# mishapadidar/GP-Derivatives-Variational-Inference

Hardware: AMD Instinct MI355X
Metric: ELBO steps/sec, DSVGP d=20 N=1M M=500 p=5 (higher is better)
Workload: dtype f32 (f64 Cholesky/solves); 1 GPU; DSVGP d=20 N=1M M=500 p=5 B=4096; global_batch=4096, per_gpu_batch=4096, M_prime=3000, parallelism=dp1 rows, trsm_nb=4096, graph_replay=False, one_call_step=True, dense_product=hand-written (gemm32.hip, v_mfma_f32_32x32x2_f32)

## Files before the change

gp-derivatives-variational-inference_amd/csrc/gemm32.hip:

```cpp
#include <cstdlib>
#include <type_traits>

#include "common.h"

namespace {

using acc16 = float __attribute__((ext_vector_type(16)));
using acc4f = float __attribute__((ext_vector_type(4)));
constexpr int TM = 128, TN = 128;

#ifndef G32_BK
#define G32_BK 32
#endif
#ifndef G32_MINW
#define G32_MINW 3
#endif
#ifndef G32_BAND
#define G32_BAND 8
#endif
#ifndef G32_DMA_BK
#define G32_DMA_BK 32
#endif
#ifndef G32_MF
#define G32_MF 32
#endif
#ifndef G32_SK_BELOW
#define G32_SK_BELOW 4096
#endif
#ifndef G32_SK_MINK
#define G32_SK_MINK 512
#endif
#ifndef G32_WIDE_ROUNDS
#define G32_WIDE_ROUNDS 3
#endif
#ifndef G32_WIDE_FILL
#define G32_WIDE_FILL 90
#endif
#ifndef G32_SK_SLOTS
#define G32_SK_SLOTS 256
#endif

struct G32 {
    const float* A; const float* B; float* C;
    int64_t lda, ldb, ldc;
    int M, N, K, tiles_m, tiles_n, flags, splitk, kslice, ntiles;
    float alpha;
    float* slab;
};

template <int BK, bool KC>
struct Stage {
    static constexpr int NV = BK / 8;
    float4 v[NV];
};

template <int BK>
struct FetchKC {
    static constexpr int CPR = BK / 4, RPP = 256 / CPR, NV = BK / 8;
    const float* P;
    int rowoff[NV];
    int kc, klim;
    __device__ __forceinline__ void init(const float* P_, int64_t ld, int mn0, int MN, int K, int tid) {
        P = P_;
        kc = (tid % CPR) * 4;
        klim = ((K + 3) / 4) * 4 - 4;
#pragma unroll
        for (int i = 0; i < NV; ++i) rowoff[i] = (int)(min(mn0 + tid / CPR + i * RPP, MN - 1) * ld);
    }
    __device__ __forceinline__ void load(int k0, int kend, Stage<BK, true>& s) const {
        const int k = k0 + kc;
        const float* p = P + min(k, klim);
#pragma unroll
        for (int i = 0; i < NV; ++i) s.v[i] = *reinterpret_cast<const float4*>(p + rowoff[i]);
        if (k0 + BK > kend) {
#pragma unroll
            for (int i = 0; i < NV; ++i) {
                s.v[i].x = (k < kend) ? s.v[i].x : 0.f;
                s.v[i].y = (k + 1 < kend) ? s.v[i].y : 0.f;
                s.v[i].z = (k + 2 < kend) ? s.v[i].z : 0.f;
                s.v[i].w = (k + 3 < kend) ? s.v[i].w : 0.f;
            }
        }
    }
};
template <int BK>
struct FetchMC {
    static constexpr int NV = BK / 8;
    const float* P;
    int64_t ld;
    int kr, K;
    __device__ __forceinline__ void init(const float* P_, int64_t ld_, int mn0, int MN, int K_, int tid) {
        ld = ld_; K = K_;
        kr = tid >> 5;
        P = P_ + min(mn0 + (tid & 31) * 4, ((MN + 3) / 4) * 4 - 4);
    }
    __device__ __forceinline__ void load(int k0, int kend, Stage<BK, false>& s) const {
#pragma unroll
        for (int i = 0; i < NV; ++i) {
            const int k = k0 + kr + 8 * i;
            s.v[i] = *reinterpret_cast<const float4*>(P + (int64_t)min(k, K - 1) * ld);
            if (k0 + BK > kend && k >= kend) s.v[i] = float4{0.f, 0.f, 0.f, 0.f};
        }
    }
};

template <int TM_ = TM, int TN_ = TN>
__device__ __forceinline__ bool pick_unit(const G32& g, int& m0, int& n0, int& kbeg, int& kend) {
    const int u = (blockIdx.x >> 3) + (blockIdx.x & 7) * ((gridDim.x + 7) >> 3);
    if (u >= g.ntiles * g.splitk) return false;
    const int slice = u / g.ntiles;
    const int t = u - slice * g.ntiles;
    int tm, tn;
    if (g.flags & DSVGP_GEMM_OUT_LOWER) {
        const int tri = min(g.tiles_m, g.tiles_n), t0 = tri * (tri + 1) / 2;
        if (t < t0) {
            tm = (int)((sqrtf(8.f * (float)t + 1.f) - 1.f) * 0.5f);
            while ((tm + 1) * (tm + 2) / 2 <= t) ++tm;
            while (tm * (tm + 1) / 2 > t) --tm;
            tn = t - tm * (tm + 1) / 2;
        } else {
            tm = tri + (t - t0) / g.tiles_n;
            tn = (t - t0) % g.tiles_n;
        }
    } else {
        const int band = t / (G32_BAND * g.tiles_m), q = t - band * G32_BAND * g.tiles_m;
        const int wcols = min(G32_BAND, g.tiles_n - band * G32_BAND);
        tm = q / wcols;
        tn = band * G32_BAND + q - tm * wcols;
    }
    m0 = tm * TM_; n0 = tn * TN_;
    kbeg = slice * g.kslice; kend = min(g.K, kbeg + g.kslice);
    return true;
}

template <int NI, int NJ>
__device__ __forceinline__ void store_tile(const G32& g, const acc16 (&acc)[NI][NJ], int m0, int n0, int wr, int wc, int h, int r,
                                           float* Cb, int64_t ldcb, bool atomic_) {
    const bool atomic = atomic_, out_lower = g.flags & DSVGP_GEMM_OUT_LOWER;
#pragma unroll
    for (int i = 0; i < NI; ++i)
#pragma unroll
        for (int j = 0; j < NJ; ++j)
#pragma unroll
            for (int c = 0; c < 16; ++c) {
                const int m = m0 + wr * (32 * NI) + i * 32 + (c & 3) + 8 * (c >> 2) + 4 * h;
                const int n = n0 + wc * (32 * NJ) + j * 32 + r;
                if (m >= g.M || n >= g.N) continue;
                if (out_lower && n > m) continue;
                const float v = g.alpha * acc[i][j][c];
                float* dst = Cb + (int64_t)m * ldcb + n;
                if (atomic) atomicAdd(dst, v);
                else *dst = v;
            }
}
#define G32_DEST()                                                                                     \
    const int slice_ = g.kslice > 0 ? kbeg / g.kslice : 0;                                             \
    float* const Cb = g.slab ? g.slab + (int64_t)slice_ * g.M * g.N : g.C;                            \
    const int64_t ldcb = g.slab ? (int64_t)g.N : g.ldc;                                                \
    const bool atomic_ = g.splitk > 1 && !g.slab

template <int BK, bool A_KC, bool B_KC>
__global__ __launch_bounds__(256, G32_MINW) void gemm32_kernel(const G32 g) {
    constexpr int SKC = BK + 2, SMC = TM + 4;
    constexpr int A_WORDS = A_KC ? TM * SKC : BK * SMC, B_WORDS = B_KC ? TN * SKC : BK * SMC;
    __shared__ __attribute__((aligned(16))) float lds[A_WORDS + B_WORDS];
    float* As = lds;
    float* Bs = lds + A_WORDS;
    const int tid = threadIdx.x, lane = tid & 63, wave = tid >> 6, wr = wave >> 1, wc = wave & 1;
    const int h = lane >> 5, r = lane & 31;
    int m0, n0, kbeg, kend;
    if (!pick_unit(g, m0, n0, kbeg, kend)) return;

    Stage<BK, A_KC> ra;
    Stage<BK, B_KC> rb;
    typename std::conditional<A_KC, FetchKC<BK>, FetchMC<BK>>::type fa;
    typename std::conditional<B_KC, FetchKC<BK>, FetchMC<BK>>::type fb;
    fa.init(g.A, g.lda, m0, g.M, g.K, tid);
    fb.init(g.B, g.ldb, n0, g.N, g.K, tid);
    auto fetch = [&](int k0) {
        fa.load(k0, kend, ra);
        fb.load(k0, kend, rb);
    };
    auto commit = [&]() {
        if constexpr (A_KC) {
            constexpr int CPR = BK / 4, RPP = 256 / CPR;
            float* p = As + (tid / CPR) * SKC + (tid % CPR) * 4;
#pragma unroll
            for (int i = 0; i < BK / 8; ++i) {
                *reinterpret_cast<float2*>(p + i * RPP * SKC) = float2{ra.v[i].x, ra.v[i].y};
                *reinterpret_cast<float2*>(p + i * RPP * SKC + 2) = float2{ra.v[i].z, ra.v[i].w};
            }
        } else {
            float* p = As + (tid >> 5) * SMC + (tid & 31) * 4;
#pragma unroll
            for (int i = 0; i < BK / 8; ++i) *reinterpret_cast<float4*>(p + 8 * i * SMC) = ra.v[i];
        }
        if constexpr (B_KC) {
            constexpr int CPR = BK / 4, RPP = 256 / CPR;
            float* p = Bs + (tid / CPR) * SKC + (tid % CPR) * 4;
#pragma unroll
            for (int i = 0; i < BK / 8; ++i) {
                *reinterpret_cast<float2*>(p + i * RPP * SKC) = float2{rb.v[i].x, rb.v[i].y};
                *reinterpret_cast<float2*>(p + i * RPP * SKC + 2) = float2{rb.v[i].z, rb.v[i].w};
            }
        } else {
            float* p = Bs + (tid >> 5) * SMC + (tid & 31) * 4;
#pragma unroll
            for (int i = 0; i < BK / 8; ++i) *reinterpret_cast<float4*>(p + 8 * i * SMC) = rb.v[i];
        }
    };

    acc16 acc[2][2];
#pragma unroll
    for (int i = 0; i < 2; ++i)
#pragma unroll
        for (int j = 0; j < 2; ++j)
#pragma unroll
            for (int c = 0; c < 16; ++c) acc[i][j][c] = 0.f;

    const float* af = A_KC ? As + (wr * 64 + r) * SKC + 2 * h : As + (2 * h) * SMC + wr * 64 + r;
    const float* bf = B_KC ? Bs + (wc * 64 + r) * SKC + 2 * h : Bs + (2 * h) * SMC + wc * 64 + r;

    if (kbeg < kend) {
        fetch(kbeg);
        for (int k0 = kbeg; k0 < kend; k0 += BK) {
            commit();
            __syncthreads();
            if (k0 + BK < kend) fetch(k0 + BK);
#pragma unroll
            for (int kk = 0; kk < BK / 4; ++kk) {
                float2 a[2], b[2];
#pragma unroll
                for (int i = 0; i < 2; ++i) {
                    if constexpr (A_KC) a[i] = *reinterpret_cast<const float2*>(af + i * 32 * SKC + 4 * kk);
                    else a[i] = float2{af[(4 * kk) * SMC + i * 32], af[(4 * kk + 1) * SMC + i * 32]};
                }
#pragma unroll
                for (int j = 0; j < 2; ++j) {
                    if constexpr (B_KC) b[j] = *reinterpret_cast<const float2*>(bf + j * 32 * SKC + 4 * kk);
                    else b[j] = float2{bf[(4 * kk) * SMC + j * 32], bf[(4 * kk + 1) * SMC + j * 32]};
                }
#pragma unroll
                for (int i = 0; i < 2; ++i)
#pragma unroll
                    for (int j = 0; j < 2; ++j) {
                        acc[i][j] = __builtin_amdgcn_mfma_f32_32x32x2f32(a[i].x, b[j].x, acc[i][j], 0, 0, 0);
                        acc[i][j] = __builtin_amdgcn_mfma_f32_32x32x2f32(a[i].y, b[j].y, acc[i][j], 0, 0, 0);
                    }
            }
            __syncthreads();
        }
    }

    G32_DEST();
    store_tile(g, acc, m0, n0, wr, wc, h, r, Cb, ldcb, atomic_);
}

#ifdef G32_STAMP
__device__ unsigned long long g32_stamps[8];
#define G32_T(var) unsigned long long var; do { __builtin_amdgcn_sched_barrier(0); \
    asm volatile("s_memtime %0\n\ts_waitcnt lgkmcnt(0)" : "=s"(var) :: "memory"); __builtin_amdgcn_sched_barrier(0); } while (0)
#else
#define G32_T(var) do { } while (0)
#endif
typedef __attribute__((address_space(3))) void* lds_ptr_t;
typedef const __attribute__((address_space(1))) void* glb_ptr_t;
__device__ __attribute__((aligned(16))) float g32_zero_chunk[4] = {0.f, 0.f, 0.f, 0.f};

__device__ __forceinline__ void lds_dma16(const float* gsrc, unsigned lds_byte_addr) {
    unsigned keep;
    asm volatile("s_mov_b32 %0, m0\n\ts_mov_b32 m0, %2\n\ts_nop 0\n\tglobal_load_lds_dwordx4 %1, off\n\ts_mov_b32 m0, %0"
                 : "=&s"(keep) : "v"(gsrc), "s"(lds_byte_addr) : "memory");
}

template <int MF, bool A_KC, bool B_KC, int BK>
__global__ __launch_bounds__(256, BK == 16 ? 3 : 2) void gemm32_dma_kernel(const G32 g) {
    static_assert(BK == 32 || (BK == 16 && MF == 32), "the 64-byte-row swizzle is derived for the 32 x 32 x 2 shape");
    constexpr int OPW = 128 * BK;
    constexpr int NP = BK / 8;
    constexpr int CH = BK / 4, RPP = 256 / BK;
    constexpr int TS = MF, NT = 64 / TS, NH = 64 / TS, NJ = BK / (4 * NH);
    __shared__ __attribute__((aligned(16))) float lds[2][2 * OPW];
    const int tid = threadIdx.x, lane = tid & 63, wave = tid >> 6, wr = wave >> 1, wc = wave & 1;
    const int h = lane / TS, r = lane % TS;
    int m0, n0, kbeg, kend;
    if (!pick_unit(g, m0, n0, kbeg, kend)) return;

    const float* asrc[NP];
    const float* bsrc[NP];
    int akk[NP], bkk[NP];
    const int K4 = (g.K + 3) / 4 * 4;
    auto swz = [](int R) { return BK == 32 ? ((R >> 1) & 7) : ((R >> 2) & 3); };
#pragma unroll
    for (int i = 0; i < NP; ++i) {
        const int blk = wave * NP + i;
        if constexpr (A_KC) {
            const int R = blk * RPP + lane / CH, c = (lane % CH) ^ swz(R);
            asrc[i] = g.A + (int64_t)min(m0 + R, g.M - 1) * g.lda + kbeg + 4 * c;
            akk[i] = 4 * c;
        } else {
            const int k = blk * 2 + (lane >> 5);
            asrc[i] = g.A + (int64_t)(kbeg + k) * g.lda + min(m0 + 4 * (lane & 31), (g.M + 3) / 4 * 4 - 4);
            akk[i] = k;
        }
        if constexpr (B_KC) {
            const int R = blk * RPP + lane / CH, c = (lane % CH) ^ swz(R);
            bsrc[i] = g.B + (int64_t)min(n0 + R, g.N - 1) * g.ldb + kbeg + 4 * c;
            bkk[i] = 4 * c;
        } else {
            const int k = blk * 2 + (lane >> 5);
            bsrc[i] = g.B + (int64_t)(kbeg + k) * g.ldb + min(n0 + 4 * (lane & 31), (g.N + 3) / 4 * 4 - 4);
            bkk[i] = k;
        }
    }
    const int64_t astep = A_KC ? BK : (int64_t)BK * g.lda, bstep = B_KC ? BK : (int64_t)BK * g.ldb;
    const unsigned lds_base = (unsigned)(uintptr_t)(lds_ptr_t)&lds[0][0];
    const unsigned wave_u = __builtin_amdgcn_readfirstlane(wave);
    auto dma = [&](int buf, int k0) {
        const unsigned dst = lds_base + (unsigned)buf * (2 * OPW * 4) + wave_u * (NP * 1024);
        const bool tail = k0 + BK > kend;
#pragma unroll
        for (int i = 0; i < NP; ++i) {
            const float* sa = asrc[i];
            const float* sb = bsrc[i];
            if (tail) {
                if (k0 + akk[i] >= (A_KC ? K4 : g.K)) sa = g32_zero_chunk;
                if (k0 + bkk[i] >= (B_KC ? K4 : g.K)) sb = g32_zero_chunk;
            }
            lds_dma16(sa, dst + i * 1024);
            lds_dma16(sb, dst + OPW * 4 + i * 1024);
            asrc[i] += astep;
            bsrc[i] += bstep;
        }
    };

    using accT = typename std::conditional<MF == 32, acc16, acc4f>::type;
    accT acc[NT][NT];
#pragma unroll
    for (int i = 0; i < NT; ++i)
#pragma unroll
        for (int j = 0; j < NT; ++j)
#pragma unroll
            for (int c = 0; c < (MF == 32 ? 16 : 4); ++c) acc[i][j][c] = 0.f;

    const int q7 = h ^ swz(r);
    int aoff[NJ], boff[NJ];
#pragma unroll
    for (int j = 0; j < NJ; ++j) {
        aoff[j] = A_KC ? (wr * 64 + r) * BK + 4 * ((NH * j) ^ q7) : (4 * NH * j + 4 * h) * 128 + wr * 64 + r;
        boff[j] = B_KC ? (wc * 64 + r) * BK + 4 * ((NH * j) ^ q7) : (4 * NH * j + 4 * h) * 128 + wc * 64 + r;
    }

    struct Frag { float a[NT][4], b[NT][4]; };
    auto load_frag = [&](const float* As, const float* Bs, int j, Frag& f) {
#pragma unroll
        for (int i = 0; i < NT; ++i) {
            if constexpr (A_KC) {
                const float4 v = *reinterpret_cast<const float4*>(As + aoff[j] + i * TS * BK);
                f.a[i][0] = v.x; f.a[i][1] = v.y; f.a[i][2] = v.z; f.a[i][3] = v.w;
            } else {
#pragma unroll
                for (int e = 0; e < 4; ++e) f.a[i][e] = As[aoff[j] + e * 128 + i * TS];
            }
            if constexpr (B_KC) {
                const float4 v = *reinterpret_cast<const float4*>(Bs + boff[j] + i * TS * BK);
                f.b[i][0] = v.x; f.b[i][1] = v.y; f.b[i][2] = v.z; f.b[i][3] = v.w;
            } else {
#pragma unroll
                for (int e = 0; e < 4; ++e) f.b[i][e] = Bs[boff[j] + e * 128 + i * TS];
            }
        }
    };

    if (kbeg < kend) {
        dma(0, kbeg);
        asm volatile("s_waitcnt vmcnt(0)" ::: "memory");
        __syncthreads();
        int buf = 0;
#ifdef G32_STAMP
        unsigned long long d_dma = 0, d_mfma = 0, d_vm = 0, d_bar = 0, n_st = 0;
#endif
        for (int k0 = kbeg; k0 < kend; k0 += BK, buf ^= 1) {
            G32_T(t0);
            if (k0 + BK < kend) dma(buf ^ 1, k0 + BK);
            G32_T(t1);
            const float* As = &lds[buf][0];
            const float* Bs = As + OPW;
            Frag f[2];
            load_frag(As, Bs, 0, f[0]);
#pragma unroll
            for (int j = 0; j < NJ; ++j) {
                if (j + 1 < NJ) load_frag(As, Bs, j + 1, f[(j + 1) & 1]);
                __builtin_amdgcn_sched_barrier(0);
                const Frag& c = f[j & 1];
#pragma unroll
                for (int e = 0; e < 4; ++e)
#pragma unroll
                    for (int i = 0; i < NT; ++i)
#pragma unroll
                        for (int jn = 0; jn < NT; ++jn) {
                            if constexpr (MF == 32)
                                acc[i][jn] = __builtin_amdgcn_mfma_f32_32x32x2f32(c.a[i][e], c.b[jn][e], acc[i][jn], 0, 0, 0);
                            else
                                acc[i][jn] = __builtin_amdgcn_mfma_f32_16x16x4f32(c.a[i][e], c.b[jn][e], acc[i][jn], 0, 0, 0);
                        }
                __builtin_amdgcn_sched_barrier(0);
            }
            G32_T(t2);
            asm volatile("s_waitcnt vmcnt(0)" ::: "memory");
            G32_T(t3);
            __syncthreads();
#ifdef G32_STAMP
            G32_T(t4);
            d_dma += t1 - t0; d_mfma += t2 - t1; d_vm += t3 - t2; d_bar += t4 - t3; ++n_st;
#endif
        }
#ifdef G32_STAMP
        if (tid == 0 && blockIdx.x == gridDim.x / 2 + 8) {
            g32_stamps[0] = d_dma; g32_stamps[1] = d_mfma; g32_stamps[2] = d_vm; g32_stamps[3] = d_bar; g32_stamps[4] = n_st;
        }
#endif
    }
    G32_DEST();
    if constexpr (MF == 32) {
        store_tile(g, acc, m0, n0, wr, wc, h, r, Cb, ldcb, atomic_);
    } else {
        const bool atomic = atomic_, out_lower = g.flags & DSVGP_GEMM_OUT_LOWER;
#pragma unroll
        for (int i = 0; i < NT; ++i)
#pragma unroll
            for (int j = 0; j < NT; ++j)
#pragma unroll
                for (int c = 0; c < 4; ++c) {
                    const int m = m0 + wr * 64 + i * 16 + 4 * h + c;
                    const int n = n0 + wc * 64 + j * 16 + r;
                    if (m >= g.M || n >= g.N) continue;
                    if (out_lower && n > m) continue;
                    const float v = g.alpha * acc[i][j][c];
                    float* dst = Cb + (int64_t)m * ldcb + n;
                    if (atomic) atomicAdd(dst, v);
                    else *dst = v;
                }
    }
}

constexpr int WTM = 256, WTN = 192, WBK = 32;
constexpr int W_AWORDS = WTM * WBK, W_BWORDS = WBK * WTN, W_STAGE = W_AWORDS + W_BWORDS;
constexpr int W_NA = W_AWORDS / 1024, W_NB = W_BWORDS / 1024;
constexpr int W_LDS_BYTES = 2 * W_STAGE * 4;

__global__ __launch_bounds__(256, 1) void gemm32_wide_kernel(const G32 g) {
    extern __shared__ __attribute__((aligned(16))) float wlds[];
    const int tid = threadIdx.x, lane = tid & 63, wave = tid >> 6, wr = wave >> 1, wc = wave & 1;
    const int h = lane >> 5, r = lane & 31;
    int m0, n0, kbeg, kend;
    if (!pick_unit<WTM, WTN>(g, m0, n0, kbeg, kend)) return;

    const float* asrc[W_NA];
    const float* bsrc[W_NB];
    int akk[W_NA], bkk[W_NB];
    const int K4 = (g.K + 3) / 4 * 4;
#pragma unroll
    for (int i = 0; i < W_NA; ++i) {
        const int R = (wave * W_NA + i) * 8 + (lane >> 3), c = (lane & 7) ^ ((R >> 1) & 7);
        asrc[i] = g.A + (int64_t)min(m0 + R, g.M - 1) * g.lda + kbeg + 4 * c;
        akk[i] = 4 * c;
    }
#pragma unroll
    for (int i = 0; i < W_NB; ++i) {
        const int ch = (wave * W_NB + i) * 64 + lane, k = ch / (WTN / 4), n4 = ch % (WTN / 4);
        bsrc[i] = g.B + (int64_t)(kbeg + k) * g.ldb + min(n0 + 4 * n4, (g.N + 3) / 4 * 4 - 4);
        bkk[i] = k;
    }
    const int64_t bstep = (int64_t)WBK * g.ldb;
    const unsigned lds_base = (unsigned)(uintptr_t)(lds_ptr_t)&wlds[0];
    const unsigned wave_u = __builtin_amdgcn_readfirstlane(wave);

    acc16 acc[4][3];
#pragma unroll
    for (int i = 0; i < 4; ++i)
#pragma unroll
        for (int j = 0; j < 3; ++j)
#pragma unroll
            for (int c = 0; c < 16; ++c) acc[i][j][c] = 0.f;

    const int q7 = h ^ ((r >> 1) & 7);
    int aoff[4];
#pragma unroll
    for (int j = 0; j < 4; ++j) aoff[j] = (wr * 128 + r) * WBK + 4 * ((2 * j) ^ q7);
    const int boff = (4 * h) * WTN + wc * 96 + r;

    auto stage = [&](auto mode_, int buf, int knext) {
        constexpr int MODE = decltype(mode_)::value;
        const float* As = wlds + buf * W_STAGE;
        const float* Bs = As + W_AWORDS;
        const unsigned dst = lds_base + (unsigned)(buf ^ 1) * (W_STAGE * 4);
        float fa[2][4][4], fb[2][3][4];
        auto rd_a = [&](int j, int i) {
            const float4 v = *reinterpret_cast<const float4*>(As + aoff[j] + i * 32 * WBK);
            fa[j & 1][i][0] = v.x; fa[j & 1][i][1] = v.y; fa[j & 1][i][2] = v.z; fa[j & 1][i][3] = v.w;
        };
        auto rd_b = [&](int j, int jn, int ep) {
#pragma unroll
            for (int e = 2 * ep; e < 2 * ep + 2; ++e) fb[j & 1][jn][e] = Bs[boff + (8 * j + e) * WTN + jn * 32];
        };
        auto dma1 = [&](int d) {
            if (d < W_NA) {
                const float* s = asrc[d];
                if (MODE == 2) s = (knext + akk[d] >= K4) ? g32_zero_chunk : s;
                lds_dma16(s, dst + (wave_u * W_NA + d) * 1024);
                asrc[d] += WBK;
            } else {
                const int i = d - W_NA;
                const float* s = bsrc[i];
                if (MODE == 2) s = (knext + bkk[i] >= g.K) ? g32_zero_chunk : s;
                lds_dma16(s, dst + W_AWORDS * 4 + (wave_u * W_NB + i) * 1024);
                bsrc[i] += bstep;
            }
        };
#pragma unroll
        for (int i = 0; i < 4; ++i) rd_a(0, i);
#pragma unroll
        for (int q = 0; q < 6; ++q) rd_b(0, q >> 1, q & 1);
#pragma unroll
        for (int j = 0; j < 4; ++j) {
            const int nd = MODE == 0 ? 0 : (j < 2 ? 5 : (j == 2 ? 4 : 0)), d0 = j < 2 ? 5 * j : 10;
#pragma unroll
            for (int n = 0; n < 48; ++n) {
                const int e = n / 12, i = (n / 3) % 4, jn = n % 3;
                acc[i][jn] = __builtin_amdgcn_mfma_f32_32x32x2f32(fa[j & 1][i][e], fb[j & 1][jn][e], acc[i][jn], 0, 0, 0);
                if (n & 1) {
                    const int t = n >> 1;
                    __builtin_amdgcn_sched_barrier(0);
                    if (t < nd) {
                        dma1(d0 + t);
                    } else if (j < 3) {
                        const int q = t - nd;
                        if (q < 4) rd_a(j + 1, q);
                        else if (q < 10) rd_b(j + 1, (q - 4) >> 1, (q - 4) & 1);
                    }
                    __builtin_amdgcn_sched_barrier(0);
                }
            }
        }
        if (MODE != 0) {
            asm volatile("s_waitcnt vmcnt(0)" ::: "memory");
            __syncthreads();
        }
    };

    if (kbeg < kend) {
        const int nst = (kend - kbeg + WBK - 1) / WBK;
        {
            const unsigned dst = lds_base;
#pragma unroll
            for (int i = 0; i < W_NA; ++i) {
                lds_dma16((kbeg + akk[i] >= K4) ? g32_zero_chunk : asrc[i], dst + (wave_u * W_NA + i) * 1024);
                asrc[i] += WBK;
            }
#pragma unroll
            for (int i = 0; i < W_NB; ++i) {
                lds_dma16((kbeg + bkk[i] >= g.K) ? g32_zero_chunk : bsrc[i], dst + W_AWORDS * 4 + (wave_u * W_NB + i) * 1024);
                bsrc[i] += bstep;
            }
        }
        asm volatile("s_waitcnt vmcnt(0)" ::: "memory");
        __syncthreads();
        int buf = 0, k0 = kbeg + WBK;
        for (int s = 0; s + 2 < nst; ++s, buf ^= 1, k0 += WBK) stage(std::integral_constant<int, 1>{}, buf, k0);
        if (nst >= 2) { stage(std::integral_constant<int, 2>{}, buf, k0); buf ^= 1; }
        stage(std::integral_constant<int, 0>{}, buf, 0);
    }
    store_tile(g, acc, m0, n0, wr, wc, h, r, g.C, g.ldc, false);
}

template <int BK>
int dispatch32(hipStream_t st, const G32& a, dim3 grid, bool akc, bool bkc) {
    if (akc && bkc) hipLaunchKernelGGL((gemm32_kernel<BK, true, true>), grid, dim3(256), 0, st, a);
    else if (akc) hipLaunchKernelGGL((gemm32_kernel<BK, true, false>), grid, dim3(256), 0, st, a);
    else if (bkc) hipLaunchKernelGGL((gemm32_kernel<BK, false, true>), grid, dim3(256), 0, st, a);
    else hipLaunchKernelGGL((gemm32_kernel<BK, false, false>), grid, dim3(256), 0, st, a);
    hipError_t e = hipGetLastError();
    return e == hipSuccess ? 1 : 1000 + (int)e;
}

}

#ifdef G32_STAMP
int g32_read_stamps(unsigned long long* out) { return (int)hipMemcpyFromSymbol(out, HIP_SYMBOL(g32_stamps), sizeof(unsigned long long) * 8); }
#endif

int launch_gemm32(hipStream_t st, const GemmArgs& g) {
    const int fl = g.flags;
    if (fl & ~(DSVGP_GEMM_TRANS_A | DSVGP_GEMM_TRANS_B | DSVGP_GEMM_OUT_LOWER | DSVGP_GEMM_K_PADDED | DSVGP_GEMM_C_ZEROED | DSVGP_GEMM_UPPER_UNDEF)) return 0;
    if (g.batch != 1 || g.splitk != 1 || g.Cin || g.kscale || g.C32 || !g.C || g.beta != 0.0) return 0;
    if (g.M < 512 || g.N < 512 || g.K < 512) return 0;
    if (g.lda % 4 || g.ldb % 4 || ((uintptr_t)g.A % 16) || ((uintptr_t)g.B % 16)) return 0;
    {
        const int64_t a_minor = (fl & DSVGP_GEMM_TRANS_A) ? g.M : g.K, b_minor = (fl & DSVGP_GEMM_TRANS_B) ? g.K : g.N;
        if (g.lda < (a_minor + 3) / 4 * 4 || g.ldb < (b_minor + 3) / 4 * 4) return 0;
        const int64_t a_rows = (fl & DSVGP_GEMM_TRANS_A) ? g.K : g.M, b_rows = (fl & DSVGP_GEMM_TRANS_B) ? g.N : g.K;
        if (a_rows * g.lda >= (int64_t)1 << 31 || b_rows * g.ldb >= (int64_t)1 << 31) return 0;
    }
    const bool out_lower = fl & DSVGP_GEMM_OUT_LOWER;
    G32 a{};
    a.A = (const float*)g.A; a.B = (const float*)g.B; a.C = (float*)g.C;
    a.lda = g.lda; a.ldb = g.ldb; a.ldc = g.ldc;
    a.M = g.M; a.N = g.N; a.K = g.K; a.flags = fl; a.alpha = (float)g.alpha;
    a.tiles_m = cdiv(g.M, TM); a.tiles_n = cdiv(g.N, TN);
    if (out_lower) {
        const int tri = a.tiles_m < a.tiles_n ? a.tiles_m : a.tiles_n;
        a.ntiles = tri * (tri + 1) / 2 + (a.tiles_m > tri ? (a.tiles_m - tri) * a.tiles_n : 0);
    } else {
        a.ntiles = a.tiles_m * a.tiles_n;
    }
    int sk = 1;
    if (a.ntiles < G32_SK_BELOW && g.K >= G32_SK_MINK) {
        double best = 1e300;
        const int maxsk = g.K / 256 < 64 ? g.K / 256 : 64;
        for (int c = 1; c <= maxsk; ++c) {
            const double tcost = (double)cdiv((int64_t)a.ntiles * c, G32_SK_SLOTS) * ((double)g.K / c + 384.0);
            if (tcost < best * 0.999) { best = tcost; sk = c; }
        }
    }
    const bool akc = !(fl & DSVGP_GEMM_TRANS_A), bkc = (fl & DSVGP_GEMM_TRANS_B) != 0;
    const bool dma_ok = !((akc || bkc) && g.K % 4 != 0 && !(g.flags & DSVGP_GEMM_K_PADDED));
    const char* wenv = getenv("DSVGP_G32_WIDE");
    const int wmode = wenv ? atoi(wenv) : 3;
    const bool wide_can = !out_lower && akc && !bkc && dma_ok && !g.slab;
    bool wide = false;
    if (wmode == 3) {
        const int64_t wt = (int64_t)cdiv(g.M, WTM) * cdiv(g.N, WTN), rounds = (wt + G32_SK_SLOTS - 1) / G32_SK_SLOTS;
        wide = wide_can && sk == 1 && wt >= (int64_t)G32_WIDE_ROUNDS * G32_SK_SLOTS && wt * 100 >= rounds * G32_SK_SLOTS * G32_WIDE_FILL;
    } else if (wmode != 0) {
        if (wmode == 2 && !wide_can) return 1000 + (int)hipErrorInvalidValue;
        if (wide_can) sk = 1;
        wide = wide_can && wmode > 0;
    }
    if (wide) {
        a.tiles_m = cdiv(g.M, WTM); a.tiles_n = cdiv(g.N, WTN);
        a.ntiles = a.tiles_m * a.tiles_n;
        a.splitk = 1;
        a.kslice = cdiv(g.K, 32) * 32;
        hipError_t e = hipFuncSetAttribute((const void*)gemm32_wide_kernel, hipFuncAttributeMaxDynamicSharedMemorySize, W_LDS_BYTES);
        if (e != hipSuccess) return 1000 + (int)e;
        hipLaunchKernelGGL(gemm32_wide_kernel, dim3(cdiv(a.ntiles, 8) * 8), dim3(256), W_LDS_BYTES, st, a);
        e = hipGetLastError();
        return e == hipSuccess ? 1 : 1000 + (int)e;
    }
    sk = slab_slices(g, sk, sizeof(float));
    a.splitk = sk;
    a.kslice = cdiv(cdiv(g.K, sk), 32) * 32;
    a.splitk = cdiv(g.K, a.kslice);
    a.slab = (g.slab && a.splitk > 1) ? (float*)g.slab : nullptr;
    if (!a.slab && (a.splitk > 1 || (out_lower && !(fl & DSVGP_GEMM_UPPER_UNDEF))) && !(fl & DSVGP_GEMM_C_ZEROED)) {
        hipError_t e = zero_block(a.C, sizeof(float), a.ldc, a.M, a.N, st);
        if (e != hipSuccess) return 1000 + (int)e;
    }
    const dim3 grid(cdiv((int64_t)a.ntiles * a.splitk, 8) * 8);
    if (dma_ok) {
        if (akc && bkc) hipLaunchKernelGGL((gemm32_dma_kernel<G32_MF, true, true, G32_DMA_BK>), grid, dim3(256), 0, st, a);
        else if (akc) hipLaunchKernelGGL((gemm32_dma_kernel<G32_MF, true, false, G32_DMA_BK>), grid, dim3(256), 0, st, a);
        else if (bkc) hipLaunchKernelGGL((gemm32_dma_kernel<G32_MF, false, true, G32_DMA_BK>), grid, dim3(256), 0, st, a);
        else hipLaunchKernelGGL((gemm32_dma_kernel<G32_MF, false, false, G32_DMA_BK>), grid, dim3(256), 0, st, a);
        hipError_t e = hipGetLastError();
        if (e != hipSuccess) return 1000 + (int)e;
    } else
    {
        const int rc = dispatch32<G32_BK>(st, a, grid, akc, bkc);
        if (rc != 1) return rc;
    }
    if (a.slab) {
        const int rc = launch_splitk_reduce(st, 0, a.slab, a.splitk, a.M, a.N, a.C, a.ldc, nullptr, 0, out_lower ? 1 : 0, 0);
        if (rc) return rc;
    }
    return 1;
}
```

Before: 85.72 steps/s.

## Add stream-K persistent 256x256 gram kernel for lower-triangular GEMM outputs

Adds a persistent kernel that handles lower-triangular (gram) products with one workgroup per CU. The linearised (tile, k-step) space is split evenly across workgroups in a stream-K walk, using 256x256 tiles with double-buffered LDS DMA. Partial tiles are combined with float atomicAdd into a pre-zeroed C, which aims to fix wave-quantisation imbalance and improve reuse over the 128x128 split-K path. The cost is atomic contention, an extra zeroing pass and non-deterministic summation order. It is on by default when the work is large enough relative to the CU count.

```diff
diff --git a/gp-derivatives-variational-inference_amd/csrc/gemm32.hip b/gp-derivatives-variational-inference_amd/csrc/gemm32.hip
--- a/gp-derivatives-variational-inference_amd/csrc/gemm32.hip
+++ b/gp-derivatives-variational-inference_amd/csrc/gemm32.hip
@@ -2,6 +2,7 @@
 #include <type_traits>
 
 #include "common.h"
+#include "gram_walk.h"
 
 namespace {
 
@@ -35,6 +36,15 @@
 #endif
 #ifndef G32_WIDE_FILL
 #define G32_WIDE_FILL 90
+#endif
+#ifndef G32_GRAM_STAGES
+#define G32_GRAM_STAGES 160
+#endif
+#ifndef G32_GRAM_INFLIGHT
+#define G32_GRAM_INFLIGHT 16
+#endif
+#ifndef G32_GRAM_KCHUNKS
+#define G32_GRAM_KCHUNKS 1
 #endif
 #ifndef G32_SK_SLOTS
 #define G32_SK_SLOTS 256
@@ -574,6 +584,159 @@
     store_tile(g, acc, m0, n0, wr, wc, h, r, g.C, g.ldc, false);
 }
 
+constexpr int GT = 256, GBK = 32;
+constexpr int G_OPWORDS = GT * GBK, G_STAGE = 2 * G_OPWORDS;
+constexpr int G_NP = G_OPWORDS / 1024;
+constexpr int G_LDS_BYTES = 2 * G_STAGE * 4;
+
+struct G32Gram {
+    const float* A; const float* B; float* C;
+    int64_t lda, ldb, ldc;
+    int M, N, K, nwg;
+    float alpha;
+    GramWalk walk;
+};
+
+__global__ __launch_bounds__(256, 1) void gemm32_gram_kernel(const G32Gram g) {
+    extern __shared__ __attribute__((aligned(16))) float glds[];
+    const int tid = threadIdx.x, lane = tid & 63, wave = tid >> 6, wr = wave >> 1, wc = wave & 1;
+    const int h = lane >> 5, r = lane & 31;
+    const int wg = gram_walk_wg(blockIdx.x, gridDim.x);
+    if (wg >= g.nwg) return;
+    long long gi, gend;
+    gram_walk_range(g.walk, wg, g.nwg, gi, gend);
+
+    const int K4 = (g.K + 3) / 4 * 4;
+    const unsigned lds_base = (unsigned)(uintptr_t)(lds_ptr_t)&glds[0];
+    const unsigned wave_u = __builtin_amdgcn_readfirstlane(wave);
+    const int q7 = h ^ ((r >> 1) & 7);
+    int aoff[4], boff[4];
+#pragma unroll
+    for (int j = 0; j < 4; ++j) {
+        aoff[j] = (wr * 128 + r) * GBK + 4 * ((2 * j) ^ q7);
+        boff[j] = (wc * 128 + r) * GBK + 4 * ((2 * j) ^ q7);
+    }
+    int drow[G_NP], dkk[G_NP];
+#pragma unroll
+    for (int i = 0; i < G_NP; ++i) {
+        drow[i] = (wave * G_NP + i) * 8 + (lane >> 3);
+        dkk[i] = 4 * ((lane & 7) ^ ((drow[i] >> 1) & 7));
+    }
+
+    while (gi < gend) {
+        const GramUnit u = gram_walk_unit(g.walk, gi, gend);
+        gi += u.s1 - u.s0;
+        const int m0 = u.tm * GT, n0 = u.tn * GT, nst = u.s1 - u.s0, kbeg = u.s0 * GBK;
+        const float* asrc[G_NP];
+        const float* bsrc[G_NP];
+#pragma unroll
+        for (int i = 0; i < G_NP; ++i) {
+            asrc[i] = g.A + (int64_t)min(m0 + drow[i], g.M - 1) * g.lda + kbeg + dkk[i];
+            bsrc[i] = g.B + (int64_t)min(n0 + drow[i], g.N - 1) * g.ldb + kbeg + dkk[i];
+        }
+        acc16 acc[4][4];
+#pragma unroll
+        for (int i = 0; i < 4; ++i)
+#pragma unroll
+            for (int j = 0; j < 4; ++j)
+#pragma unroll
+                for (int c = 0; c < 16; ++c) acc[i][j][c] = 0.f;
+
+        auto stage = [&](auto mode_, int buf, int knext) {
+            constexpr int MODE = decltype(mode_)::value;
+            const float* As = glds + buf * G_STAGE;
+            const float* Bs = As + G_OPWORDS;
+            const unsigned dst = lds_base + (unsigned)(buf ^ 1) * (G_STAGE * 4);
+            float fa[2][4][4], fb[2][4][4];
+            auto rd_a = [&](int j, int i) {
+                const float4 v = *reinterpret_cast<const float4*>(As + aoff[j] + i * 32 * GBK);
+                fa[j & 1][i][0] = v.x; fa[j & 1][i][1] = v.y; fa[j & 1][i][2] = v.z; fa[j & 1][i][3] = v.w;
+            };
+            auto rd_b = [&](int j, int i) {
+                const float4 v = *reinterpret_cast<const float4*>(Bs + boff[j] + i * 32 * GBK);
+                fb[j & 1][i][0] = v.x; fb[j & 1][i][1] = v.y; fb[j & 1][i][2] = v.z; fb[j & 1][i][3] = v.w;
+            };
+            auto dma1 = [&](int d) {
+                if (d < G_NP) {
+                    const float* s = asrc[d];
+                    if (MODE == 2) s = (knext + dkk[d] >= K4) ? g32_zero_chunk : s;
+                    lds_dma16(s, dst + (wave_u * G_NP + d) * 1024);
+                    asrc[d] += GBK;
+                } else {
+                    const int i = d - G_NP;
+                    const float* s = bsrc[i];
+                    if (MODE == 2) s = (knext + dkk[i] >= K4) ? g32_zero_chunk : s;
+                    lds_dma16(s, dst + G_OPWORDS * 4 + (wave_u * G_NP + i) * 1024);
+                    bsrc[i] += GBK;
+                }
+            };
+#pragma unroll
+            for (int i = 0; i < 4; ++i) rd_a(0, i);
+#pragma unroll
+            for (int i = 0; i < 4; ++i) rd_b(0, i);
+#pragma unroll
+            for (int j = 0; j < 4; ++j) {
+                const int nd = MODE == 0 ? 0 : (j == 0 ? 6 : (j < 3 ? 5 : 0)), d0 = j == 0 ? 0 : (j == 1 ? 6 : 11);
+#pragma unroll
+                for (int n = 0; n < 64; ++n) {
+                    const int e = n / 16, i = (n / 4) % 4, jn = n % 4;
+                    acc[i][jn] = __builtin_amdgcn_mfma_f32_32x32x2f32(fa[j & 1][i][e], fb[j & 1][jn][e], acc[i][jn], 0, 0, 0);
+                    if (n & 1) {
+                        const int t = n >> 1;
+                        __builtin_amdgcn_sched_barrier(0);
+                        if (t < nd) {
+                            dma1(d0 + t);
+                        } else if (j < 3) {
+                            const int q = t - nd;
+                            if (q < 4) rd_a(j + 1, q);
+                            else if (q < 8) rd_b(j + 1, q - 4);
+                        }
+                        __builtin_amdgcn_sched_barrier(0);
+                    }
+                }
+            }
+            if (MODE != 0) {
+                asm volatile("s_waitcnt vmcnt(0)" ::: "memory");
+                __syncthreads();
+            }
+        };
+
+        __syncthreads();
+        {
+#pragma unroll
+            for (int i = 0; i < G_NP; ++i) {
+                const bool z = kbeg + dkk[i] >= K4;
+                lds_dma16(z ? g32_zero_chunk : asrc[i], lds_base + (wave_u * G_NP + i) * 1024);
+                lds_dma16(z ? g32_zero_chunk : bsrc[i], lds_base + G_OPWORDS * 4 + (wave_u * G_NP + i) * 1024);
+                asrc[i] += GBK;
+                bsrc[i] += GBK;
+            }
+        }
+        asm volatile("s_waitcnt vmcnt(0)" ::: "memory");
+        __syncthreads();
+        int buf = 0, k0 = kbeg + GBK;
+        for (int s = 0; s + 2 < nst; ++s, buf ^= 1, k0 += GBK) stage(std::integral_constant<int, 1>{}, buf, k0);
+        if (nst >= 2) { stage(std::integral_constant<int, 2>{}, buf, k0); buf ^= 1; }
+        stage(std::integral_constant<int, 0>{}, buf, 0);
+
+#pragma unroll
+        for (int i = 0; i < 4; ++i)
+#pragma unroll
+            for (int j = 0; j < 4; ++j) {
+                const int mt = m0 + wr * 128 + i * 32, nt = n0 + wc * 128 + j * 32;
+                if (mt >= g.M || nt >= g.N || nt > mt + 31) continue;
+                const int n = nt + r;
+                float* dst = g.C + (int64_t)(mt + 4 * h) * g.ldc + n;
+#pragma unroll
+                for (int c = 0; c < 16; ++c) {
+                    const int mo = (c & 3) + 8 * (c >> 2), m = mt + 4 * h + mo;
+                    if (m < g.M && n < g.N && n <= m) atomicAdd(dst + (int64_t)mo * g.ldc, g.alpha * acc[i][j][c]);
+                }
+                if (G32_GRAM_INFLIGHT < 63) asm volatile("s_waitcnt vmcnt(%0)" ::"n"(G32_GRAM_INFLIGHT) : "memory");
+            }
+    }
+}
+
 template <int BK>
 int dispatch32(hipStream_t st, const G32& a, dim3 grid, bool akc, bool bkc) {
     if (akc && bkc) hipLaunchKernelGGL((gemm32_kernel<BK, true, true>), grid, dim3(256), 0, st, a);
@@ -592,15 +755,18 @@
 
 int launch_gemm32(hipStream_t st, const GemmArgs& g) {
     const int fl = g.flags;
-    if (fl & ~(DSVGP_GEMM_TRANS_A | DSVGP_GEMM_TRANS_B | DSVGP_GEMM_OUT_LOWER | DSVGP_GEMM_K_PADDED | DSVGP_GEMM_C_ZEROED | DSVGP_GEMM_UPPER_UNDEF)) return 0;
-    if (g.batch != 1 || g.splitk != 1 || g.Cin || g.kscale || g.C32 || !g.C || g.beta != 0.0) return 0;
-    if (g.M < 512 || g.N < 512 || g.K < 512) return 0;
-    if (g.lda % 4 || g.ldb % 4 || ((uintptr_t)g.A % 16) || ((uintptr_t)g.B % 16)) return 0;
+    const char* genv = getenv("DSVGP_G32_GRAM");
+    const int gmode = genv ? atoi(genv) : 3;
+    const int not_taken = (gmode == 2 && (fl & DSVGP_GEMM_OUT_LOWER)) ? 1000 + (int)hipErrorInvalidValue : 0;
+    if (fl & ~(DSVGP_GEMM_TRANS_A | DSVGP_GEMM_TRANS_B | DSVGP_GEMM_OUT_LOWER | DSVGP_GEMM_K_PADDED | DSVGP_GEMM_C_ZEROED | DSVGP_GEMM_UPPER_UNDEF)) return not_taken;
+    if (g.batch != 1 || g.splitk != 1 || g.Cin || g.kscale || g.C32 || !g.C || g.beta != 0.0) return not_taken;
+    if (g.M < 512 || g.N < 512 || g.K < 512) return not_taken;
+    if (g.lda % 4 || g.ldb % 4 || ((uintptr_t)g.A % 16) || ((uintptr_t)g.B % 16)) return not_taken;
     {
         const int64_t a_minor = (fl & DSVGP_GEMM_TRANS_A) ? g.M : g.K, b_minor = (fl & DSVGP_GEMM_TRANS_B) ? g.K : g.N;
-        if (g.lda < (a_minor + 3) / 4 * 4 || g.ldb < (b_minor + 3) / 4 * 4) return 0;
+        if (g.lda < (a_minor + 3) / 4 * 4 || g.ldb < (b_minor + 3) / 4 * 4) return not_taken;
         const int64_t a_rows = (fl & DSVGP_GEMM_TRANS_A) ? g.K : g.M, b_rows = (fl & DSVGP_GEMM_TRANS_B) ? g.N : g.K;
-        if (a_rows * g.lda >= (int64_t)1 << 31 || b_rows * g.ldb >= (int64_t)1 << 31) return 0;
+        if (a_rows * g.lda >= (int64_t)1 << 31 || b_rows * g.ldb >= (int64_t)1 << 31) return not_taken;
     }
     const bool out_lower = fl & DSVGP_GEMM_OUT_LOWER;
     G32 a{};
@@ -648,6 +814,37 @@
         e = hipGetLastError();
         return e == hipSuccess ? 1 : 1000 + (int)e;
     }
+    const bool gram_can = out_lower && akc && bkc && dma_ok && !g.slab;
+    if (gmode == 2 && out_lower && !gram_can) return 1000 + (int)hipErrorInvalidValue;
+    if (gram_can && gmode != 0) {
+        static int cus[64];
+        int dev = 0;
+        hipError_t e = hipGetDevice(&dev);
+        if (e != hipSuccess) return 1000 + (int)e;
+        int ncu = (dev >= 0 && dev < 64) ? cus[dev] : 0;
+        if (ncu <= 0) {
+            e = hipDeviceGetAttribute(&ncu, hipDeviceAttributeMultiprocessorCount, dev);
+            if (e != hipSuccess || ncu <= 0) return 1000 + (int)(e != hipSuccess ? e : hipErrorInvalidValue);
+            if (dev >= 0 && dev < 64) cus[dev] = ncu;
+        }
+        const char* cenv = getenv("DSVGP_G32_GRAM_KCHUNKS");
+        const int kchunks = cenv ? atoi(cenv) : G32_GRAM_KCHUNKS;
+        G32Gram w{};
+        w.walk = gram_walk_make(g.M, g.N, g.K, GT, GBK, kchunks);
+        if (gmode != 3 || w.walk.G >= (long long)G32_GRAM_STAGES * ncu) {
+            w.A = a.A; w.B = a.B; w.C = a.C; w.lda = g.lda; w.ldb = g.ldb; w.ldc = g.ldc;
+            w.M = g.M; w.N = g.N; w.K = g.K; w.nwg = ncu; w.alpha = a.alpha;
+            if (!(fl & DSVGP_GEMM_C_ZEROED)) {
+                e = zero_block(a.C, sizeof(float), a.ldc, a.M, a.N, st);
+                if (e != hipSuccess) return 1000 + (int)e;
+            }
+            e = hipFuncSetAttribute((const void*)gemm32_gram_kernel, hipFuncAttributeMaxDynamicSharedMemorySize, G_LDS_BYTES);
+            if (e != hipSuccess) return 1000 + (int)e;
+            hipLaunchKernelGGL(gemm32_gram_kernel, dim3(cdiv(ncu, 8) * 8), dim3(256), G_LDS_BYTES, st, w);
+            e = hipGetLastError();
+            return e == hipSuccess ? 1 : 1000 + (int)e;
+        }
+    }
     sk = slab_slices(g, sk, sizeof(float));
     a.splitk = sk;
     a.kslice = cdiv(cdiv(g.K, sk), 32) * 32;
diff --git a/gp-derivatives-variational-inference_amd/csrc/gram_walk.h b/gp-derivatives-variational-inference_amd/csrc/gram_walk.h
--- /dev/null
+++ b/gp-derivatives-variational-inference_amd/csrc/gram_walk.h
@@ -0,0 +1,66 @@
+#pragma once
+#include <math.h>
+
+#if defined(__HIPCC__)
+#define GRAM_WALK_FN __host__ __device__ __forceinline__
+#else
+#define GRAM_WALK_FN inline
+#endif
+
+struct GramWalk {
+    int tiles_m, tiles_n, ntiles;
+    int S, Sc, nchunk;
+    long long G;
+};
+struct GramUnit { int tm, tn, s0, s1; };
+
+GRAM_WALK_FN GramWalk gram_walk_make(int M, int N, int K, int tile, int bk, int kchunks) {
+    GramWalk w;
+    w.tiles_m = (M + tile - 1) / tile;
+    w.tiles_n = (N + tile - 1) / tile;
+    const int tri = w.tiles_m < w.tiles_n ? w.tiles_m : w.tiles_n;
+    w.ntiles = tri * (tri + 1) / 2 + (w.tiles_m > tri ? (w.tiles_m - tri) * w.tiles_n : 0);
+    w.S = (K + bk - 1) / bk;
+    if (kchunks < 1) kchunks = 1;
+    w.Sc = (w.S + kchunks - 1) / kchunks;
+    if (w.Sc < 1) w.Sc = 1;
+    w.nchunk = (w.S + w.Sc - 1) / w.Sc;
+    w.G = (long long)w.ntiles * w.S;
+    return w;
+}
+
+GRAM_WALK_FN void gram_walk_tile(const GramWalk& w, int t, int& tm, int& tn) {
+    const int tri = w.tiles_m < w.tiles_n ? w.tiles_m : w.tiles_n, t0 = tri * (tri + 1) / 2;
+    if (t < t0) {
+        tm = (int)((sqrtf(8.f * (float)t + 1.f) - 1.f) * 0.5f);
+        while ((tm + 1) * (tm + 2) / 2 <= t) ++tm;
+        while (tm * (tm + 1) / 2 > t) --tm;
+        tn = t - tm * (tm + 1) / 2;
+    } else {
+        tm = tri + (t - t0) / w.tiles_n;
+        tn = (t - t0) % w.tiles_n;
+    }
+}
+
+GRAM_WALK_FN int gram_walk_wg(int block, int grid) { return (block >> 3) + (block & 7) * (grid >> 3); }
+
+GRAM_WALK_FN void gram_walk_range(const GramWalk& w, int wg, int nwg, long long& g0, long long& g1) {
+    g0 = (long long)wg * w.G / nwg;
+    g1 = (long long)(wg + 1) * w.G / nwg;
+}
+
+GRAM_WALK_FN GramUnit gram_walk_unit(const GramWalk& w, long long g, long long g1) {
+    const long long per = (long long)w.ntiles * w.Sc;
+    int c = (int)(g / per);
+    if (c > w.nchunk - 1) c = w.nchunk - 1;
+    const long long rem = g - (long long)c * per;
+    const int len = c == w.nchunk - 1 ? w.S - c * w.Sc : w.Sc;
+    const int t = (int)(rem / len), sl = (int)(rem - (long long)t * len);
+    long long n = len - sl;
+    if (n > g1 - g) n = g1 - g;
+    GramUnit u;
+    gram_walk_tile(w, t, u.tm, u.tn);
+    u.s0 = c * w.Sc + sl;
+    u.s1 = u.s0 + (int)n;
+    return u;
+}
```

After: 87.92 steps/s, median of 6. 1.03x the previous value.
